# nkwangyh/CubemapSLAM

Hardware: AMD Instinct MI355X
Metric: frames/sec (extract+match+localBA) on Lafida cam0 (higher is better)
Workload: dtype u8 (extract/match), f64 (BA)

## Files before the change

### cubemapslam_amd/csrc/cms_api_ba_lm.hip

```cpp

struct BaLm {
  int iterations = 0, robust = 0;
  double delta = 0;
  int it = 0, qmax = 0, nBad = 0, done = 0, next = 0;
  double lambda = -1, ni = 2, currentChi = 0, iniChi = 0, rho = 0;
  double chi_ini = 0, chi_fin = 0, lam_fin = 0;
};

static bool ba_stopped(const volatile uint8_t* stop) { return stop && *stop; }

static int ba_enqueue_iter_start(cms_ba* b, const BaLm& st) {
  hipStream_t s = b->stream;
  const int cur = b->cur;
  ba_errors(b, cur, st.robust, st.delta, 0);
  hipLaunchKernelGGL(k_ba_lin_points, dim3(b->nblk_p), dim3(128), 0, s, b->d, (const double*)b->d_poses[cur],
                     (const double*)b->d_pts[cur], st.robust, st.delta, b->d_Hll, b->d_bl, b->d_Hpl);
  hipLaunchKernelGGL(k_ba_lin_poses, dim3(b->K, BA_POSE_CHUNKS), dim3(256), 0, s, b->d, (const double*)b->d_poses[cur],
                     (const double*)b->d_pts[cur], st.robust, st.delta, b->d_pose_partial);
  if (b->np > 0)
    hipLaunchKernelGGL(k_ba_pose_finish, dim3(b->np), dim3(64), 0, s, b->np, (const double*)b->d_pose_partial, b->d_Hpp, b->d_bp);
  if (st.it == 0) {
    HIPCHK(hipMemsetAsync(b->d_scal + 3, 0, sizeof(double), s));
    hipLaunchKernelGGL(k_ba_maxdiag, dim3(64), dim3(256), 0, s, b->np, b->P, (const double*)b->d_Hpp, (const double*)b->d_Hll, b->d_scal + 3);
  }
  HIPCHK(hipMemcpyAsync(b->h_pin, b->d_scal, 4 * sizeof(double), hipMemcpyDeviceToHost, s));
  return CMS_OK;
}
static void ba_finish_iter_start(cms_ba* b, BaLm& st) {
  st.currentChi = b->h_pin[0];
  st.iniChi = st.currentChi;
  if (st.it == 0) { st.chi_ini = st.iniChi; st.lambda = 1e-5 * b->h_pin[3]; st.ni = 2; st.nBad = 0; }
  st.rho = 0; st.qmax = 0;
// ... 95 lines not shown
      ++nact;
    }
    if (nact == 0) break;
    for (int w = 0; w < n; ++w) {
      if (stepped[w] < 0) continue;
      HIPCHK(hipStreamSynchronize(bas[w]->stream));
      if (stepped[w] == 0) ba_finish_iter_start(bas[w], st[w]);
      else ba_finish_trial(bas[w], st[w], stop);
    }
  }
  HIPCHK(hipGetLastError());
  return CMS_OK;
}

static bool ba_can_batch(cms_ba** bas, int n) {
  const bool single_old = ba_knobs().single_host_lm;
  if (n < (single_old ? 2 : 1) || n > BA_MAX_GROUP) return false;
  for (int w = 0; w < n; ++w) if (!bas[w]->solve_blk || bas[w]->device != bas[0]->device) return false;
  return true;
}
static int ba_group_reserve(cms_ba* owner, int n) {
  if (owner->grp_cap >= n) return CMS_OK;
  if (owner->grp_items_host) ba_pin_give(owner->device, owner->grp_items_host, owner->grp_pin_bytes[0]);
  if (owner->grp_scal_host) ba_pin_give(owner->device, owner->grp_scal_host, owner->grp_pin_bytes[1]);
  if (owner->grp_lm_host) ba_pin_give(owner->device, owner->grp_lm_host, owner->grp_pin_bytes[2]);
  owner->grp_items_host = nullptr; owner->grp_scal_host = nullptr; owner->grp_lm_host = nullptr;
  owner->grp_cap = 0;
  const int cap = std::max(n, 8);
  { char* q = nullptr; int rc = ba_alloc(owner, &q, (size_t)cap * sizeof(BaItem)); if (rc) return rc; owner->grp_items_dev = q; }
  { int rc = ba_alloc(owner, &owner->grp_scal_dev, (size_t)cap * 8); if (rc) return rc; }
  { char* q = nullptr; int rc = ba_alloc(owner, &q, (size_t)cap * sizeof(BaLmDev)); if (rc) return rc; owner->grp_lm_dev = q; }
  HIPCHK(ba_pin_take(owner->device, (size_t)cap * sizeof(BaItem), &owner->grp_items_host, &owner->grp_pin_bytes[0]));
  HIPCHK(ba_pin_take(owner->device, (size_t)cap * 8 * sizeof(double), (void**)&owner->grp_scal_host, &owner->grp_pin_bytes[1]));
  HIPCHK(ba_pin_take(owner->device, (size_t)cap * sizeof(BaLmDev), &owner->grp_lm_host, &owner->grp_pin_bytes[2]));
  n = cap;
  owner->grp_cap = n;
  return CMS_OK;
}
static bool ba_all_sp(cms_ba** bas, int n) {
  for (int w = 0; w < n; ++w) if (bas[w]->sp.R <= 0) return false;
  return true;
}
static bool ba_use_se(cms_ba** bas, int n) {
  if (ba_knobs().host_lm) return false;
  for (int w = 0; w < n; ++w) if (bas[w]->se.nchunks <= 0 || bas[w]->det_points) return false;
  return true;
}
static bool ba_use_te(cms_ba** bas, int n) {
  if (ba_knobs().trial_points || !ba_use_se(bas, n)) return false;
  for (int w = 0; w < n; ++w) if (bas[w]->se.Rt <= 0) return false;
  return true;
}
static int ba_device_cus(int dev) {
  static std::mutex mu;
  static int cus_of[64] = {0};
  int cus = 256;
  std::lock_guard<std::mutex> lk(mu);
  if (dev >= 0 && dev < 64) {
    if (cus_of[dev] == 0) { hipDeviceProp_t pr; cus_of[dev] = hipGetDeviceProperties(&pr, dev) == hipSuccess && pr.multiProcessorCount > 0 ? pr.multiProcessorCount : 256; }
    cus = cus_of[dev];
  }
  return cus;
}
static int ba_group_ranges(cms_ba** bas, int n) {
  const int cus = ba_device_cus(bas[0]->device);
  int R = BA_SE_RANGES;
  static const int reserve = [] { const char* v = getenv("CMS_BA_RESERVE_CUS"); return v ? std::max(0, atoi(v)) : 0; }();
// ... 64 lines not shown
        HIPCHK(hipMemsetAsync(b->d_se_bp_partial, 0, (size_t)b->np * 6 * sizeof(double), g->stream));
      }
      b->gsum_clean = false;
    }
  }
  static_assert(sizeof(BaItem) % 16 == 0, "BaItem is copied in 16-byte words");
  static const bool items_by_copy_engine = getenv("CMS_BA_ITEMS_COPY_ENGINE") != nullptr;
  if (items_by_copy_engine) HIPCHK(hipMemcpyAsync(g->grp_items_dev, items, (size_t)n * sizeof(BaItem), hipMemcpyHostToDevice, g->stream));
  else {
    const int n16 = (int)((size_t)n * sizeof(BaItem) / 16);
    hipLaunchKernelGGL(k_copy16, dim3((n16 + 63) / 64), dim3(64), 0, g->stream, (uint4*)g->grp_items_dev, (const uint4*)items, n16);
  }
  HIPCHK(hipGetLastError());
  return CMS_OK;
}
static int ba_optimize_stage_batched(cms_ba** bas, int n, std::vector<BaLm>& st, const volatile uint8_t* stop) {
  cms_ba* g = bas[0];
  hipStream_t s = g->stream;
  const BaItem* ditems = reinterpret_cast<const BaItem*>(g->grp_items_dev);
  int max_e = 0, max_p = 0, max_K = 0, max_np = 0, max_chunks = 0, max_P = 0, max_R = 0, max_spt = 64, max_pairs = 0;
  size_t lds = 0, sp_lds = 0;
  const bool all_sp = ba_all_sp(bas, n);
  for (int w = 0; w < n; ++w) {
    max_R = std::max(max_R, bas[w]->sp.R); max_spt = std::max(max_spt, bas[w]->sp_threads); max_pairs = std::max(max_pairs, bas[w]->npairs);
    sp_lds = std::max(sp_lds, bas[w]->sp_lds);
    max_e = std::max(max_e, bas[w]->nblk_e); max_p = std::max(max_p, bas[w]->nblk_p); max_K = std::max(max_K, bas[w]->K);
    max_np = std::max(max_np, bas[w]->np); max_chunks = std::max(max_chunks, bas[w]->nchunks); max_P = std::max(max_P, bas[w]->P);
    lds = std::max(lds, bas[w]->blk_lds);
  }
  int rc = CMS_OK;
  {
    BaLmDev* hlm0 = reinterpret_cast<BaLmDev*>(g->grp_lm_host);
    for (int w = 0; w < n; ++w) memset(&hlm0[w], 0, sizeof(BaLmDev));
    hipLaunchKernelGGL(kb_ba_lm_load, dim3((n + 63) / 64), dim3(64), 0, s, ditems, n, st[0].robust ? 1 : 0);
  }
  BaDyn dyn{};
  memset(&dyn, 0, sizeof(dyn));
  dyn.robust = st[0].robust; dyn.delta = st[0].delta; dyn.chi2_th = 5.991; dyn.set_level = 0;
  for (;;) {
    int n_iter = 0, n_trial = 0;
    for (int w = 0; w < n; ++w) {
      dyn.phase[w] = BA_PHASE_IDLE;
      if (st[w].next == 0 && (st[w].it >= st[w].iterations || ba_stopped(stop))) st[w].next = 2;
      if (st[w].next == 0) { dyn.phase[w] = BA_PHASE_ITER; ++n_iter; }
      else if (st[w].next == 1) { dyn.phase[w] = BA_PHASE_TRIAL; ++n_trial; }
      dyn.cur[w] = (uint8_t)bas[w]->cur; dyn.first_iter[w] = st[w].it == 0; dyn.lambda[w] = st[w].lambda;
    }
    if (n_iter + n_trial == 0) break;
    if (n_iter) {
      hipLaunchKernelGGL(kb_ba_errors, dim3(max_e, 1, n), dim3(256), 0, s, ditems, dyn, (int)BA_PHASE_ITER);
      hipLaunchKernelGGL(kb_ba_reduce, dim3(1, 1, n), dim3(256), 0, s, ditems, dyn, (int)BA_PHASE_ITER);
      hipLaunchKernelGGL(kb_ba_lin_points, dim3(max_p, 1, n), dim3(128), 0, s, ditems, dyn, (int)BA_PHASE_ITER);
      hipLaunchKernelGGL(kb_ba_lin_poses, dim3(max_K, BA_POSE_CHUNKS, n), dim3(256), 0, s, ditems, dyn, (int)BA_PHASE_ITER);
      hipLaunchKernelGGL(kb_ba_pose_finish, dim3(std::max(max_np, 1), 1, n), dim3(64), 0, s, ditems, dyn, (int)BA_PHASE_ITER);
      hipLaunchKernelGGL(kb_ba_maxdiag, dim3(1, 1, n), dim3(1024), 0, s, ditems, dyn, (int)BA_PHASE_ITER);
    }
    if (n_trial) {
      if (!all_sp)
        hipLaunchKernelGGL(kb_ba_dinv, dim3((max_P + 255) / 256, 1, n), dim3(256), 0, s, ditems, dyn, (int)BA_PHASE_TRIAL);
      if (all_sp) {
        hipLaunchKernelGGL(kb_ba_schur_points, dim3(max_R, 1, n), dim3(max_spt), sp_lds, s, ditems, dyn, (int)BA_PHASE_TRIAL);
        hipLaunchKernelGGL(kb_ba_schur_reduce, dim3(max_pairs, 1, n), dim3(256), 0, s, ditems, dyn, (int)BA_PHASE_TRIAL);
      } else if (max_chunks > 0) {
        hipLaunchKernelGGL(kb_ba_schur_chunks, dim3(max_chunks, 1, n), dim3(256), 0, s, ditems, dyn, (int)BA_PHASE_TRIAL);
      }
      hipLaunchKernelGGL(kb_ba_trial_solve, dim3(1, 1, n), dim3(384), lds, s, ditems, dyn, (int)BA_PHASE_TRIAL);
      hipLaunchKernelGGL(kb_ba_trial_points, dim3(max_p, 1, n), dim3(128), 0, s, ditems, dyn, (int)BA_PHASE_TRIAL);
      hipLaunchKernelGGL(kb_ba_reduce2, dim3(1, 1, n), dim3(256), 0, s, ditems, dyn, (int)BA_PHASE_TRIAL);
    }
    HIPCHK(hipStreamSynchronize(s));
    for (int w = 0; w < n; ++w) {
      if (dyn.phase[w] == BA_PHASE_IDLE) continue;
      memcpy(bas[w]->h_pin, g->grp_scal_host + 8 * w, 8 * sizeof(double));
      if (dyn.phase[w] == BA_PHASE_ITER) ba_finish_iter_start(bas[w], st[w]);
      else ba_finish_trial(bas[w], st[w], stop);
    }
  }
  HIPCHK(hipGetLastError());
  return CMS_OK;
}
static int ba_optimize_stage_batched_dev(cms_ba** bas, int n, std::vector<BaLm>& st, const volatile uint8_t* stop) {
  cms_ba* g = bas[0];
  hipStream_t s = g->stream;
  const BaItem* ditems = reinterpret_cast<const BaItem*>(g->grp_items_dev);
  int max_e = 0, max_p = 0, max_K = 0, max_np = 0, max_chunks = 0, max_P = 0, max_R = 0, max_spt = 64, max_pairs = 0, max_it = 0;
  size_t lds = 0, sp_lds = 0;
  const bool all_sp = ba_all_sp(bas, n);
  for (int w = 0; w < n; ++w) {
    max_R = std::max(max_R, bas[w]->sp.R); max_spt = std::max(max_spt, bas[w]->sp_threads); max_pairs = std::max(max_pairs, bas[w]->npairs);
    sp_lds = std::max(sp_lds, bas[w]->sp_lds);
    max_e = std::max(max_e, bas[w]->nblk_e); max_p = std::max(max_p, bas[w]->nblk_p); max_K = std::max(max_K, bas[w]->K);
    max_np = std::max(max_np, bas[w]->np); max_chunks = std::max(max_chunks, bas[w]->nchunks); max_P = std::max(max_P, bas[w]->P);
    lds = std::max(lds, bas[w]->blk_lds);
    max_it = std::max(max_it, st[w].iterations);
  }
  BaLmDev* hlm = reinterpret_cast<BaLmDev*>(g->grp_lm_host);
  for (int w = 0; w < n; ++w) {
    BaLmDev& L = hlm[w];
    memset(&L, 0, sizeof(L));
    L.lambda = st[w].lambda; L.ni = st[w].ni; L.it = st[w].it; L.iterations = st[w].iterations; L.nBad = st[w].nBad; L.done = st[w].done;
    L.cur = bas[w]->cur;
    L.next = (st[w].it >= st[w].iterations || ba_stopped(stop)) ? 2 : 0;
  }
  hipLaunchKernelGGL(kb_ba_lm_load, dim3((n + 63) / 64), dim3(64), 0, s, ditems, n, st[0].robust ? 1 : 0);
  BaDyn dyn{};
  memset(&dyn, 0, sizeof(dyn));
  dyn.robust = st[0].robust; dyn.delta = st[0].delta; dyn.chi2_th = 5.991; dyn.set_level = 0; dyn.dev_lm = 1; dyn.fold_finish = 1;
  bool first_round = false;
  for (int w = 0; w < n; ++w) first_round = first_round || st[w].it == 0;
  const BaGroupMode gm = ba_group_mode(bas, n);
  const bool use_se = gm.use_se, use_te = gm.use_te;
  bool iter_phase = true;
  const bool use_s3 = gm.use_s3;
  int s3_threads = 64; size_t lds3 = 0;
  for (int w = 0; w < n; ++w) { s3_threads = std::max(s3_threads, ba_s3_threads(bas[w]->np)); lds3 = std::max(lds3, bas[w]->blk3_lds); }
  {
    static const int solve_kb = [] { const char* v = getenv("CMS_BA_SOLVE_LDS_KB"); return v ? atoi(v) : 0; }();
    if (solve_kb > 0) lds3 = std::max(lds3, std::min((size_t)solve_kb * 1024, (size_t)BA_LDS_CEILING));
  }
  int max_seR = 0, max_np2 = 0, max_Rt = 0; size_t se_lds = 0, te_lds = 0, rm_lds = 0;
  const int se_waves = gm.se_waves;
  bool any_runs = false, any_rw0 = false, any_rw1 = false;
  for (int w = 0; w < n; ++w) {
    const BaSe& gs = bas[w]->grp_se;
    if (gm.run_wg) { any_rw0 = any_rw0 || gs.n_rmA > 0; any_rw1 = any_rw1 || gs.n_rm > gs.n_rmA; }
    max_seR = std::max(max_seR, gs.R_rm + gs.R); max_np2 = std::max(max_np2, gs.npairs2); se_lds = std::max(se_lds, bas[w]->se_lds_fixed);
    any_runs = any_runs || gs.R_rm > 0;
    if (gs.R_rm > 0) rm_lds = std::max(rm_lds, bas[w]->rm_lds);
    max_Rt = std::max(max_Rt, gs.Rt); te_lds = std::max(te_lds, ((size_t)24 * bas[w]->K + 6 * (size_t)std::max(bas[w]->np, 1)) * sizeof(double));
  }
  se_lds += (size_t)se_waves * ((size_t)64 * 18 * sizeof(double) + 64 * sizeof(int));
  se_lds = std::max(se_lds, rm_lds);
  const int se_threads = 64 * se_waves;
  const size_t rw_lds = ba_rw_lds(std::max(max_K, 1));
  const int rw_units0 = std::max(8, std::min(BA_RW_CUTS, ba_device_cus(bas[0]->device) * ba_knobs().rw_waves_cu0 / std::max(n, 1)));
  const int rw_units1 = std::max(8, std::min(BA_RW_CUTS, ba_device_cus(bas[0]->device) * ba_knobs().rw_waves_cu1 / std::max(n, 1)));
  const bool fused = gm.fused;
  const bool solve_reduces = fused && (gm.gsum || (!ba_knobs().separate_reduce && max_seR <= ba_knobs().solve_reduce_max));
  dyn.fused_lin = fused ? 1 : 0;
  {
    static const bool no_presum = getenv("CMS_BA_NO_SOLVE_PRESUM") != nullptr;
    const size_t need = lds3 + (size_t)max_np2 * 42 * sizeof(double);
    if (use_s3 && solve_reduces && !gm.gsum && !no_presum && need <= BA_LDS_CEILING) { dyn.solve_presum = 1; lds3 = need; }
  }
  const bool first_pass = fused && use_te && first_round && !ba_knobs().separate_first_pass;
  dyn.fold_reduce = (use_te && !ba_knobs().separate_reduce2 && ba_knobs().dup == 0) ? 1 : 0;
  int k = 0;
  const int pk = g->prof_kernel;
  const int dup = ba_knobs().dup;
  auto bracket = [&](int id, int which) {
    if (pk != id) return;
    const size_t i = 2 * (size_t)k + which;
    while (g->prof_ev.size() <= i) { hipEvent_t e = nullptr; if (hipEventCreate(&e) != hipSuccess) return; g->prof_ev.push_back(e); }
    hipEventRecord(g->prof_ev[i], s);
  };
  auto enqueue_round = [&]() {
      if (first_round && first_pass) {
        bracket(1, 0);
        hipLaunchKernelGGL(kb_ba_first_pass, dim3(max_Rt, 1, n), dim3(BA_TE_THREADS), te_lds, s, ditems, dyn, (int)BA_PHASE_ITER);
        bracket(1, 1);
        iter_phase = false;
      } else if (first_round) {
        hipLaunchKernelGGL(kb_ba_errors, dim3(max_e, 1, n), dim3(256), 0, s, ditems, dyn, (int)BA_PHASE_ITER);
        hipLaunchKernelGGL(kb_ba_reduce, dim3(1, 1, n), dim3(256), 0, s, ditems, dyn, (int)BA_PHASE_ITER);
      }
      first_round = false;
      if (iter_phase) {
        const int npb = (max_P + 255) / 256;
        bracket(1, 0);
        hipLaunchKernelGGL(kb_ba_lin, dim3(npb + max_K * BA_POSE_CHUNKS, 1, n), dim3(256), 0, s, ditems, dyn, (int)BA_PHASE_ITER, npb);
        if (dup == 1) hipLaunchKernelGGL(kb_ba_lin, dim3(npb + max_K * BA_POSE_CHUNKS, 1, n), dim3(256), 0, s, ditems, dyn, (int)BA_PHASE_ITER, npb);
        bracket(1, 1);
        bracket(2, 0);
        hipLaunchKernelGGL(kb_ba_maxdiag, dim3(1, 1, n), dim3(1024), 0, s, ditems, dyn, (int)BA_PHASE_ITER);
        bracket(2, 1);
      }
      if (fused) iter_phase = false;
      if (!all_sp && !use_se)
        hipLaunchKernelGGL(kb_ba_dinv, dim3((max_P + 255) / 256, 1, n), dim3(256), 0, s, ditems, dyn, (int)BA_PHASE_TRIAL);
      if (use_se) {
// ... 33 lines not shown
        bracket(4, 1);
      } else if (max_chunks > 0) {
        hipLaunchKernelGGL(kb_ba_schur_chunks, dim3(max_chunks, 1, n), dim3(256), 0, s, ditems, dyn, (int)BA_PHASE_TRIAL);
      }
      bracket(5, 0);
      if (use_s3 && solve_reduces && dyn.solve_presum) {
        hipLaunchKernelGGL(kb_ba_trial_solve3rp, dim3(1, 1, n), dim3(s3_threads), lds3, s, ditems, dyn, (int)BA_PHASE_TRIAL);
      } else if (use_s3 && solve_reduces) {
        hipLaunchKernelGGL(kb_ba_trial_solve3r, dim3(1, 1, n), dim3(s3_threads), lds3, s, ditems, dyn, (int)BA_PHASE_TRIAL);
        if (dup == 5) hipLaunchKernelGGL(kb_ba_trial_solve3r, dim3(1, 1, n), dim3(s3_threads), lds3, s, ditems, dyn, (int)BA_PHASE_TRIAL);
      } else if (use_s3) {
        hipLaunchKernelGGL(kb_ba_trial_solve3, dim3(1, 1, n), dim3(s3_threads), lds3, s, ditems, dyn, (int)BA_PHASE_TRIAL);
        if (dup == 5) hipLaunchKernelGGL(kb_ba_trial_solve3, dim3(1, 1, n), dim3(s3_threads), lds3, s, ditems, dyn, (int)BA_PHASE_TRIAL);
      } else {
        hipLaunchKernelGGL(kb_ba_trial_solve, dim3(1, 1, n), dim3(384), lds, s, ditems, dyn, (int)BA_PHASE_TRIAL);
        if (dup == 5) hipLaunchKernelGGL(kb_ba_trial_solve, dim3(1, 1, n), dim3(384), lds, s, ditems, dyn, (int)BA_PHASE_TRIAL);
      }
      bracket(5, 1);
      bracket(6, 0);
      if (use_te) {
        hipLaunchKernelGGL(kb_ba_trial_edges, dim3(max_Rt, 1, n), dim3(BA_TE_THREADS), te_lds, s, ditems, dyn, (int)BA_PHASE_TRIAL);
        if (dup == 6) hipLaunchKernelGGL(kb_ba_trial_edges, dim3(max_Rt, 1, n), dim3(BA_TE_THREADS), te_lds, s, ditems, dyn, (int)BA_PHASE_TRIAL);
      } else {
        hipLaunchKernelGGL(kb_ba_trial_points, dim3(max_p, 1, n), dim3(128), 0, s, ditems, dyn, (int)BA_PHASE_TRIAL);
        if (dup == 6) hipLaunchKernelGGL(kb_ba_trial_points, dim3(max_p, 1, n), dim3(128), 0, s, ditems, dyn, (int)BA_PHASE_TRIAL);
      }
      bracket(6, 1);
      bracket(7, 0);
      if (!dyn.fold_reduce) hipLaunchKernelGGL(kb_ba_reduce2, dim3(1, 1, n), dim3(256), 0, s, ditems, dyn, (int)BA_PHASE_TRIAL);
      bracket(7, 1);
      ++k;
  };
  const volatile BaLmDev* vh = reinterpret_cast<const volatile BaLmDev*>(hlm);
  hipError_t werr = hipSuccess;
  for (long spins = 0;;) {
    bool any = false;
    for (int w = 0; w < n; ++w) any = any || vh[w].next != 2;
    if (!any || (k > 0 && ba_stopped(stop))) break;
    if (k - vh[0].rounds < (stop ? 1 : 2)) { enqueue_round(); spins = 0; continue; }
    if (spins < 256) std::this_thread::yield();
    else std::this_thread::sleep_for(std::chrono::microseconds(20));
    if ((++spins & 0xFFF) == 0 && hipStreamQuery(s) != hipErrorNotReady) {
      werr = hipStreamSynchronize(s);
      if (werr != hipSuccess || k - vh[0].rounds >= 2) { if (werr == hipSuccess) werr = hipErrorUnknown; break; }
    }
  }
  const hipError_t serr = hipStreamSynchronize(s);
  HIPCHK(werr);
  HIPCHK(serr);
  HIPCHK(hipGetLastError());
  if (pk > 0)
    for (int r = 0; r < k && 2 * (size_t)r + 1 < g->prof_ev.size(); ++r) {
      float ms = 0;
      if (hipEventElapsedTime(&ms, g->prof_ev[2 * r], g->prof_ev[2 * r + 1]) == hipSuccess) { g->prof_ms += ms; ++g->prof_launches; }
    }
  for (int w = 0; w < n; ++w) {
    const BaLmDev& L = hlm[w];
    BaLm& t = st[w];
    t.lambda = L.lambda; t.ni = L.ni; t.currentChi = L.currentChi; t.iniChi = L.iniChi; t.rho = L.rho; t.it = L.it; t.qmax = L.qmax;
    t.nBad = L.nBad; t.done = L.done; t.next = 2;
    if (L.done > 0 || L.it > 0) { t.chi_ini = L.chi_ini; t.chi_fin = L.chi_fin; t.lam_fin = L.lam_fin; }
    if (L.next == 1 && L.qmax > 0 && ba_stopped(stop)) {
      ++t.done; t.chi_ini = L.chi_ini; t.chi_fin = L.currentChi; t.lam_fin = L.lambda;
    }
    bas[w]->cur = L.cur;
  }
  return CMS_OK;
}

static int ba_classify_batched(cms_ba** bas, int n, int set_level, std::vector<int>& counts) {
  cms_ba* g = bas[0];
  hipStream_t s = g->stream;
  BaDyn dyn{};
  memset(&dyn, 0, sizeof(dyn));
  dyn.chi2_th = 5.991; dyn.set_level = set_level;
  int max_e = 0;
  for (int w = 0; w < n; ++w) {
    dyn.phase[w] = BA_PHASE_CLASSIFY; dyn.cur[w] = (uint8_t)bas[w]->cur;
    max_e = std::max(max_e, bas[w]->nblk_e);
  }
  const BaItem* ditems = reinterpret_cast<const BaItem*>(g->grp_items_dev);
  hipLaunchKernelGGL(kb_ba_classify, dim3(max_e, 1, n), dim3(256), 0, s, ditems, dyn, (int)BA_PHASE_CLASSIFY);
  hipLaunchKernelGGL(kb_ba_counts_publish, dim3((n + 63) / 64), dim3(64), 0, s, ditems, n);
  HIPCHK(hipStreamSynchronize(s));
  const BaLmDev* hlm = reinterpret_cast<const BaLmDev*>(g->grp_lm_host);
  counts.resize(n);
  for (int w = 0; w < n; ++w) counts[w] = hlm[w].n_out[set_level ? 0 : 1];
  return CMS_OK;
}

static int ba_optimize_group(cms_ba** bas, int n, int its_robust, int its_final, const volatile uint8_t* stop, cms_ba_stats* stats);
extern "C" int cms_ba_optimize_many(cms_ba** bas, int n, int its_robust, int its_final, const volatile uint8_t* stop, cms_ba_stats* stats) {
  if (!bas || n < 1) return cms_fail(CMS_ERR_ARG, "cms_ba_optimize_many: bad argument");
  for (int w = 0; w < n; ++w) if (!bas[w]) return cms_fail(CMS_ERR_ARG, "null ba");
  auto kind = [&](int w) {
    const cms_ba* b = bas[w];
    int k = b->device * 8 + (b->fast_plan ? 4 : 0) + (b->se.nchunks > 0 ? 2 : 0) + (b->deterministic ? 1 : 0);
    if (b->deterministic) k += 1024 * (1 + (b->det_points ? 1 : 0) + 2 * (b->rm_lds > 0 ? 1 : 0) + 4 * std::max(0, std::min(15, b->se_waves)) + 64 * b->det_ranges);
    return k;
  };
  bool one = n <= BA_MAX_GROUP;
  for (int w = 1; w < n && one; ++w) one = kind(w) == kind(0);
  if (one) return ba_optimize_group(bas, n, its_robust, its_final, stop, stats);
  std::vector<char> done(n, 0);
  int rc_all = CMS_OK;
  for (int w0 = 0; w0 < n; ++w0) {
    if (done[w0]) continue;
    std::vector<cms_ba*> grp; std::vector<int> idx;
    for (int w = w0; w < n && (int)grp.size() < BA_MAX_GROUP; ++w)
      if (!done[w] && kind(w) == kind(w0)) { grp.push_back(bas[w]); idx.push_back(w); done[w] = 1; }
    std::vector<cms_ba_stats> gs(grp.size());
    const int rc = ba_optimize_group(grp.data(), (int)grp.size(), its_robust, its_final, stop, gs.data());
    if (stats) for (size_t i = 0; i < idx.size(); ++i) stats[idx[i]] = gs[i];
    if (rc < 0) return rc;
    if (rc != CMS_OK) rc_all = rc;
  }
  return rc_all;
// ... 11 lines not shown
  };
  for (int w = 0; w < n; ++w) { HIPCHK(hipSetDevice(bas[w]->device)); HIPCHK(ba_order_behind_setup(bas[w])); }
  if (!batched)
    for (int w = 0; w < n; ++w)
      if (bas[w]->async_pending) { HIPCHK(ba_wait_stream(bas[w]->stream)); bas[w]->async_pending = false; }
  if (batched) {
    HIPCHK(hipSetDevice(bas[0]->device));
    for (int w = 0; w < n; ++w) {
      if (bas[w]->async_pending && bas[w]->stream != bas[0]->stream) { HIPCHK(ba_wait_stream(bas[w]->stream)); bas[w]->async_pending = false; }
    }
    if (bas[0]->async_pending && bas[0]->own_stream) { HIPCHK(ba_wait_stream(bas[0]->stream)); bas[0]->async_pending = false; }
    tick("uploads-waited");
    int rcg = ba_group_reserve(bas[0], n);
    if (rcg) return rcg;
    rcg = ba_upload_items(bas, n);
    if (rcg) return rcg;
    for (int w = 0; w < n; ++w) { bas[w]->async_pending = true; bas[w]->grp_stream = bas[0]->stream; }
    tick("items");
  }
  std::vector<cms_ba_stats> local(n);
  for (int w = 0; w < n; ++w) memset(&local[w], 0, sizeof(cms_ba_stats));
  if (ba_stopped(stop)) {
    if (batched) for (int w = 0; w < n; ++w) bas[w]->gsum_clean = bas[w]->grp_se.gsum != 0;
    if (stats) memcpy(stats, local.data(), n * sizeof(cms_ba_stats));
    return 1;
  }
  const double delta = std::sqrt(5.991);
  std::vector<BaLm> st(n);
  for (int w = 0; w < n; ++w) { st[w] = BaLm(); st[w].iterations = its_robust; st[w].robust = 1; st[w].delta = delta; }
  const bool host_lm = ba_knobs().host_lm;
  for (int w = 0; w < n; ++w)
    if (bas[w]->se_only && (!batched || host_lm || !ba_use_se(bas, n)))
      return cms_fail(CMS_ERR_UNSUPPORTED, "cms_ba_optimize: the window carries only the edge-major work list but another kernel path was selected");
  int rc = batched ? (host_lm ? ba_optimize_stage_batched(bas, n, st, stop) : ba_optimize_stage_batched_dev(bas, n, st, stop)) : ba_optimize_stage_many(bas, n, st, stop);
  if (rc) return rc;
  tick("stage1");
  for (int w = 0; w < n; ++w) {
    local[w].iterations_done[0] = st[w].done; local[w].chi2_initial[0] = st[w].chi_ini; local[w].chi2_final[0] = st[w].chi_fin;
    local[w].lambda_final[0] = st[w].lam_fin;
  }
  std::vector<std::vector<uint8_t>> flags(n);
  std::vector<int> counts(n, 0);
  auto classify = [&](int set_level) -> int {
    if (batched) return ba_classify_batched(bas, n, set_level, counts);
    for (int w = 0; w < n; ++w) {
      cms_ba* b = bas[w];
      HIPCHK(hipSetDevice(b->device));
      flags[w].resize(b->E);
      hipLaunchKernelGGL(k_ba_classify, dim3(b->nblk_e), dim3(256), 0, b->stream, b->d, (const double*)b->d_poses[b->cur],
                         (const double*)b->d_pts[b->cur], 5.991, set_level, b->d_flags);
      HIPCHK(hipMemcpyAsync(flags[w].data(), b->d_flags, b->E, hipMemcpyDeviceToHost, b->stream));
    }
    for (int w = 0; w < n; ++w) HIPCHK(hipStreamSynchronize(bas[w]->stream));
    for (int w = 0; w < n; ++w) { counts[w] = 0; for (int e = 0; e < bas[w]->E; ++e) counts[w] += flags[w][e]; }
    return CMS_OK;
  };
  if (!ba_stopped(stop)) {
    rc = classify(1);
    if (rc) return rc;
    for (int w = 0; w < n; ++w) local[w].n_outliers_mid = counts[w];
    tick("classified");
    for (int w = 0; w < n; ++w) { st[w] = BaLm(); st[w].iterations = its_final; st[w].robust = 0; st[w].delta = delta; }
    rc = batched ? (host_lm ? ba_optimize_stage_batched(bas, n, st, stop) : ba_optimize_stage_batched_dev(bas, n, st, stop)) : ba_optimize_stage_many(bas, n, st, stop);
    if (rc) return rc;
    for (int w = 0; w < n; ++w) {
      local[w].iterations_done[1] = st[w].done; local[w].chi2_initial[1] = st[w].chi_ini; local[w].chi2_final[1] = st[w].chi_fin;
      local[w].lambda_final[1] = st[w].lam_fin;
    }
    tick("stage2");
  }
  rc = classify(0);
  if (rc) return rc;
  tick("classified");
  if (call_timing) fprintf(stderr, "[cms_ba_optimize_many] %d windows:%s\n", n, t_log.c_str());
  for (int w = 0; w < n; ++w) local[w].n_outliers_final = counts[w];
  if (stats) memcpy(stats, local.data(), n * sizeof(cms_ba_stats));
  if (batched)
    for (int w = 0; w < n; ++w) { bas[w]->async_pending = false; bas[w]->grp_stream = nullptr; bas[w]->gsum_clean = bas[w]->grp_se.gsum != 0; }
  return CMS_OK;
}

extern "C" int cms_ba_optimize(cms_ba* b, int its_robust, int its_final, const volatile uint8_t* stop, cms_ba_stats* st) {
  if (!b) return cms_fail(CMS_ERR_ARG, "null ba");
  return cms_ba_optimize_many(&b, 1, its_robust, its_final, stop, st);
}
```

### cubemapslam_amd/csrc/cms_ba_wrappers.hip

```cpp
#include <hip/hip_runtime.h>
#include <stdint.h>

#define BA_MAX_GROUP 64
struct BaLmDev {
  double lambda, ni, currentChi, iniChi, rho, chi_ini, chi_fin, lam_fin;
  int it, iterations, qmax, nBad, done, next, cur, rounds;
  int n_out[2], pad[2];
};
struct BaItem {
  BaDev d;
  double* poses[2]; double* pts[2];
  double* Hll; double* bl; double* Hpl; double* Hpp; double* bp; double* pose_partial; double* Dinv; double* db;
  double* chunk_sum; double* x; double* partial; double* scal;
  double* hscal;
  const int2* chunk_range; const int2* tup; const int* pair_of_block; const int* pair_chunk_off;
  uint8_t* flags;
  int nblk_e, nblk_p, nchunks, block_free;
  BaSp sp;
  BaSe se;
  BaLmDev* lm; BaLmDev* hlm;
};
template <class T> struct BaGP {
  BA_AS1 T* p;
  __device__ __forceinline__ BaGP() {}
  __device__ __forceinline__ BaGP(T* q) : p((BA_AS1 T*)q) {}
  __device__ __forceinline__ operator T*() const { return (T*)p; }
  __device__ __forceinline__ BA_AS1 T& operator[](size_t i) const { return p[i]; }
  __device__ __forceinline__ BA_AS1 T* operator->() const { return p; }
};
struct BaGP2 {
  BaGP<double> a, b;
  __device__ __forceinline__ BaGP<double> operator[](int i) const { BaGP<double> r; r.p = i ? b.p : a.p; return r; }
};
struct BaItemG {
  BaDevG d;
  BaGP2 poses, pts;
  BaGP<double> Hll, bl, Hpl, Hpp, bp, pose_partial, Dinv, db, chunk_sum, x, partial, scal, hscal;
  BaGP<const int2> chunk_range, tup;
  BaGP<const int> pair_of_block, pair_chunk_off;
  BaGP<uint8_t> flags;
  int nblk_e, nblk_p, nchunks, block_free;
  BaSpG sp; BaSeG se;
  BaGP<BaLmDev> lm, hlm;
  __device__ __forceinline__ BaItemG(const BaItem& t)
      : d(t.d), Hll(t.Hll), bl(t.bl), Hpl(t.Hpl), Hpp(t.Hpp), bp(t.bp), pose_partial(t.pose_partial), Dinv(t.Dinv), db(t.db), chunk_sum(t.chunk_sum), x(t.x),
        partial(t.partial), scal(t.scal), hscal(t.hscal), chunk_range(t.chunk_range), tup(t.tup), pair_of_block(t.pair_of_block),
        pair_chunk_off(t.pair_chunk_off), flags(t.flags), nblk_e(t.nblk_e), nblk_p(t.nblk_p), nchunks(t.nchunks), block_free(t.block_free), sp(t.sp), se(t.se),
        lm(t.lm), hlm(t.hlm) {
    poses.a = BaGP<double>(t.poses[0]); poses.b = BaGP<double>(t.poses[1]); pts.a = BaGP<double>(t.pts[0]); pts.b = BaGP<double>(t.pts[1]);
  }
};
struct BaDyn {
  double lambda[BA_MAX_GROUP];
  uint8_t phase[BA_MAX_GROUP], cur[BA_MAX_GROUP], first_iter[BA_MAX_GROUP];
  int robust, set_level;
  double delta, chi2_th;
  int dev_lm, fold_finish;
  int fused_lin, fold_reduce;
  int solve_presum, pad_;
};
enum { BA_PHASE_IDLE = 0, BA_PHASE_ITER = 1, BA_PHASE_TRIAL = 2, BA_PHASE_CLASSIFY = 3 };

extern "C" __global__ void __launch_bounds__(256)
k_ba_errors(BaDev d, const double* poses, const double* pts, int robust, double delta, double* partial) {
  ba_errors_body(blockIdx.x, gridDim.x, d, poses, pts, robust, delta, partial);
}
extern "C" __global__ void __launch_bounds__(256)
k_ba_reduce(const double* partial, int n, double* out, int add) { ba_reduce_body(blockIdx.x, gridDim.x, partial, n, out, add); }
extern "C" __global__ void __launch_bounds__(128)
k_ba_lin_points(BaDev d, const double* poses, const double* pts, int robust, double delta, double* Hll, double* bl, double* Hpl) {
  ba_lin_points_body(blockIdx.x, gridDim.x, d, poses, pts, robust, delta, Hll, bl, Hpl);
}
extern "C" __global__ void __launch_bounds__(256)
k_ba_lin_poses(BaDev d, const double* poses, const double* pts, int robust, double delta, double* pose_partial) {
  ba_lin_poses_body(blockIdx.x, gridDim.x, d, poses, pts, robust, delta, pose_partial);
}
extern "C" __global__ void __launch_bounds__(64)
k_ba_pose_finish(int np, const double* pose_partial, double* Hpp, double* bp) { ba_pose_finish_body(blockIdx.x, gridDim.x, np, pose_partial, Hpp, bp); }
extern "C" __global__ void __launch_bounds__(256)
k_ba_maxdiag(int np, int P, const double* Hpp, const double* Hll, double* out) { ba_maxdiag_body(blockIdx.x, gridDim.x, np, P, Hpp, Hll, out); }
extern "C" __global__ void __launch_bounds__(256)
k_ba_dinv(int P, const double* Hll, const double* bl, double lambda, double* Dinv, double* db) {
  ba_dinv_body(blockIdx.x, gridDim.x, P, Hll, bl, lambda, Dinv, db);
}
extern "C" __global__ void __launch_bounds__(256)
k_ba_schur_chunks(BaDev d, const int2* chunk_range, const int2* tup, const double* Hpl, const double* Dinv, const double* db, double* chunk_sum) {
  ba_schur_chunks_body(blockIdx.x, gridDim.x, d, chunk_range, tup, Hpl, Dinv, db, chunk_sum);
}
extern "C" __global__ void __launch_bounds__(BA_SP_MAX_THREADS + BA_SP_STAGERS) __attribute__((amdgpu_waves_per_eu(1, 3)))
k_ba_schur_points(BaDev d, BaSp sp, const double* Hpl, const double* Dinv, const double* db) { ba_schur_points_body(blockIdx.x, d, sp, Hpl, Dinv, db); }
extern "C" __global__ void __launch_bounds__(256)
k_ba_schur_reduce(BaSp sp, double* pair_sum) { ba_schur_reduce_body(blockIdx.x, sp, pair_sum); }
// ... 285 lines not shown
    for (int i = threadIdx.x; i < 6 * it.d.np; i += blockDim.x) {
      double sum = 0.0;
      for (int r = 0; r < n; ++r)
        sum += __longlong_as_double((long long)__hip_atomic_load(reinterpret_cast<BA_AS1 unsigned long long*>(it.se.partial) + ((size_t)r * 6 * it.d.np + i), __ATOMIC_RELAXED, __HIP_MEMORY_SCOPE_AGENT));
      m = fmax(m, fabs(sum));
    }
  } else
  for (int i = threadIdx.x; i < 6 * it.d.np; i += blockDim.x)
    m = fmax(m, fabs(__longlong_as_double((long long)__hip_atomic_exchange(reinterpret_cast<unsigned long long*>(pose_diag + i), 0ull, __ATOMIC_RELAXED, __HIP_MEMORY_SCOPE_AGENT))));
  if (threadIdx.x == 0) m = fmax(m, __longlong_as_double((long long)atomicExch(pt_max, 0ull)));
  for (int o = 32; o > 0; o >>= 1) m = fmax(m, __shfl_xor(m, o));
  __syncthreads();
  if ((threadIdx.x & 63) == 0) sh2[threadIdx.x >> 6] = m;
  __syncthreads();
  if (threadIdx.x == 0) {
    double mx = 0;
    for (int i = 0; i < (int)(blockDim.x >> 6); ++i) mx = fmax(mx, sh2[i]);
    it.scal[0] = chi; it.hscal[0] = chi; it.scal[3] = mx; it.hscal[3] = mx;
    atomicExch(ticket, 0);
    if (dyn.dev_lm) ba_lm_after_iter(it.lm, it.hlm, chi, mx);
  }
}
__device__ __forceinline__ void kb_ba_reduce2_window(const BaItem* __restrict__ items, const BaDyn& dyn, int phase) {
  BA_ITEM(phase, 1)
  ba_reduce2_body(0, 1, it.partial, it.se.Rt > 0 ? it.se.Rt : it.nblk_p, it.scal, it.hscal);
  ba_trial_publish(it, dyn);
}
extern "C" __global__ void __launch_bounds__(256) kb_ba_reduce2(const BaItem* __restrict__ items, BaDyn dyn, int phase) {
  kb_ba_reduce2_window(items, dyn, phase);
  if (dyn.dev_lm && blockIdx.z == 0 && threadIdx.x == 0) ba_round_count(items);
}
extern "C" __global__ void __launch_bounds__(256) kb_ba_classify(const BaItem* __restrict__ items, BaDyn dyn, int phase) {
  BA_ITEM(phase, it.nblk_e)
  ba_classify_body(blockIdx.x, it.nblk_e, it.d, it.poses[cur], it.pts[cur], dyn.chi2_th, dyn.set_level, it.flags);
  const int e = blockIdx.x * blockDim.x + threadIdx.x;
  const int n = __syncthreads_count(e < it.d.E && it.flags[e] != 0);
  if (threadIdx.x == 0 && n > 0) atomicAdd((int*)&it.lm->n_out[dyn.set_level ? 0 : 1], n);
}
extern "C" __global__ void __launch_bounds__(64) kb_ba_lm_load(const BaItem* __restrict__ items, int n, int clear_counts) {
  const int w = blockIdx.x * blockDim.x + threadIdx.x;
  if (w >= n) return;
  BaLmDev L = *items[w].hlm;
  const BaLmDev old = *items[w].lm;
  L.n_out[0] = clear_counts ? 0 : old.n_out[0];
  L.n_out[1] = clear_counts ? 0 : old.n_out[1];
  *items[w].lm = L;
  reinterpret_cast<int*>(items[w].scal + 7)[0] = 0;
  items[w].scal[6] = 0.0;
  for (int i = 0; i < 6 * items[w].d.np; ++i) items[w].Hpp[i] = 0.0;
}
extern "C" __global__ void __launch_bounds__(64) kb_ba_counts_publish(const BaItem* __restrict__ items, int n) {
  const int w = blockIdx.x * blockDim.x + threadIdx.x;
  if (w >= n) return;
  items[w].hlm->n_out[0] = items[w].lm->n_out[0];
  items[w].hlm->n_out[1] = items[w].lm->n_out[1];
}
```

Measured before the change: 25110.

## Chain BA stage 1, classify and stage 2 on device without host sync

Stage 1 of the device-driven LM loop no longer ends with a host synchronize. Outlier classification is enqueued directly behind it, and stage 2 is started from a staged host snapshot through kb_ba_lm_load, so the GPU keeps running across the stage boundary. A new round-decision helper limits how many speculative rounds are queued, using remaining iterations and a drained/confirm state, which cuts redundant trailing rounds. The cost is more complex host-device state handoff: stage flags, snapshot buffers, and pinned memory three times larger, with some risk of races in the stage handoff.

```diff
diff --git a/cubemapslam_amd/csrc/cms_api_ba_lm.hip b/cubemapslam_amd/csrc/cms_api_ba_lm.hip
--- a/cubemapslam_amd/csrc/cms_api_ba_lm.hip
+++ b/cubemapslam_amd/csrc/cms_api_ba_lm.hip
@@ -1,3 +1,4 @@
+#include "cms_ba_round_bound.h"
 
 struct BaLm {
   int iterations = 0, robust = 0;
@@ -159,7 +160,7 @@
   { char* q = nullptr; int rc = ba_alloc(owner, &q, (size_t)cap * sizeof(BaLmDev)); if (rc) return rc; owner->grp_lm_dev = q; }
   HIPCHK(ba_pin_take(owner->device, (size_t)cap * sizeof(BaItem), &owner->grp_items_host, &owner->grp_pin_bytes[0]));
   HIPCHK(ba_pin_take(owner->device, (size_t)cap * 8 * sizeof(double), (void**)&owner->grp_scal_host, &owner->grp_pin_bytes[1]));
-  HIPCHK(ba_pin_take(owner->device, (size_t)cap * sizeof(BaLmDev), &owner->grp_lm_host, &owner->grp_pin_bytes[2]));
+  HIPCHK(ba_pin_take(owner->device, (size_t)3 * cap * sizeof(BaLmDev), &owner->grp_lm_host, &owner->grp_pin_bytes[2]));
   n = cap;
   owner->grp_cap = n;
   return CMS_OK;
@@ -290,13 +291,13 @@
   {
     BaLmDev* hlm0 = reinterpret_cast<BaLmDev*>(g->grp_lm_host);
     for (int w = 0; w < n; ++w) memset(&hlm0[w], 0, sizeof(BaLmDev));
-    hipLaunchKernelGGL(kb_ba_lm_load, dim3((n + 63) / 64), dim3(64), 0, s, ditems, n, st[0].robust ? 1 : 0);
+    hipLaunchKernelGGL(kb_ba_lm_load, dim3((n + 63) / 64), dim3(64), 0, s, ditems, n, st[0].robust ? 1 : 0, (const BaLmDev*)nullptr);
   }
   BaDyn dyn{};
   memset(&dyn, 0, sizeof(dyn));
   dyn.robust = st[0].robust; dyn.delta = st[0].delta; dyn.chi2_th = 5.991; dyn.set_level = 0;
   for (;;) {
-    int n_iter = 0, n_trial = 0;
+    int n_iter = 0, n_trial = 0, n_timed = 0;
     for (int w = 0; w < n; ++w) {
       dyn.phase[w] = BA_PHASE_IDLE;
       if (st[w].next == 0 && (st[w].it >= st[w].iterations || ba_stopped(stop))) st[w].next = 2;
@@ -316,17 +317,27 @@
     if (n_trial) {
       if (!all_sp)
         hipLaunchKernelGGL(kb_ba_dinv, dim3((max_P + 255) / 256, 1, n), dim3(256), 0, s, ditems, dyn, (int)BA_PHASE_TRIAL);
+      const bool timed = g->prof_kernel == 3 && (all_sp || max_chunks > 0);
+      if (timed) {
+        while (g->prof_ev.size() < 2) { hipEvent_t e = nullptr; HIPCHK(hipEventCreate(&e)); g->prof_ev.push_back(e); }
+        hipEventRecord(g->prof_ev[0], s);
+      }
       if (all_sp) {
         hipLaunchKernelGGL(kb_ba_schur_points, dim3(max_R, 1, n), dim3(max_spt), sp_lds, s, ditems, dyn, (int)BA_PHASE_TRIAL);
         hipLaunchKernelGGL(kb_ba_schur_reduce, dim3(max_pairs, 1, n), dim3(256), 0, s, ditems, dyn, (int)BA_PHASE_TRIAL);
       } else if (max_chunks > 0) {
         hipLaunchKernelGGL(kb_ba_schur_chunks, dim3(max_chunks, 1, n), dim3(256), 0, s, ditems, dyn, (int)BA_PHASE_TRIAL);
       }
+      if (timed) { hipEventRecord(g->prof_ev[1], s); n_timed = 1; }
       hipLaunchKernelGGL(kb_ba_trial_solve, dim3(1, 1, n), dim3(384), lds, s, ditems, dyn, (int)BA_PHASE_TRIAL);
       hipLaunchKernelGGL(kb_ba_trial_points, dim3(max_p, 1, n), dim3(128), 0, s, ditems, dyn, (int)BA_PHASE_TRIAL);
       hipLaunchKernelGGL(kb_ba_reduce2, dim3(1, 1, n), dim3(256), 0, s, ditems, dyn, (int)BA_PHASE_TRIAL);
     }
     HIPCHK(hipStreamSynchronize(s));
+    if (n_timed) {
+      float ms = 0;
+      if (hipEventElapsedTime(&ms, g->prof_ev[0], g->prof_ev[1]) == hipSuccess) { g->prof_ms += ms; ++g->prof_launches; }
+    }
     for (int w = 0; w < n; ++w) {
       if (dyn.phase[w] == BA_PHASE_IDLE) continue;
       memcpy(bas[w]->h_pin, g->grp_scal_host + 8 * w, 8 * sizeof(double));
@@ -337,7 +348,13 @@
   HIPCHK(hipGetLastError());
   return CMS_OK;
 }
-static int ba_optimize_stage_batched_dev(cms_ba** bas, int n, std::vector<BaLm>& st, const volatile uint8_t* stop) {
+struct BaChain {
+  int phase = 0;
+  int k0 = 0;
+  bool chained = false;
+};
+static int ba_classify_enqueue(cms_ba** bas, int n, int set_level, bool cur_from_lm, BaLmDev* snap);
+static int ba_optimize_stage_batched_dev(cms_ba** bas, int n, std::vector<BaLm>& st, const volatile uint8_t* stop, BaChain* ch = nullptr) {
   cms_ba* g = bas[0];
   hipStream_t s = g->stream;
   const BaItem* ditems = reinterpret_cast<const BaItem*>(g->grp_items_dev);
@@ -353,14 +370,19 @@
     max_it = std::max(max_it, st[w].iterations);
   }
   BaLmDev* hlm = reinterpret_cast<BaLmDev*>(g->grp_lm_host);
+  const bool ch2 = ch && ch->phase == 2;
+  BaLmDev* start = ch2 ? hlm + g->grp_cap : hlm;
+  std::vector<int> next0(n);
   for (int w = 0; w < n; ++w) {
-    BaLmDev& L = hlm[w];
+    BaLmDev& L = start[w];
     memset(&L, 0, sizeof(L));
     L.lambda = st[w].lambda; L.ni = st[w].ni; L.it = st[w].it; L.iterations = st[w].iterations; L.nBad = st[w].nBad; L.done = st[w].done;
     L.cur = bas[w]->cur;
     L.next = (st[w].it >= st[w].iterations || ba_stopped(stop)) ? 2 : 0;
-  }
-  hipLaunchKernelGGL(kb_ba_lm_load, dim3((n + 63) / 64), dim3(64), 0, s, ditems, n, st[0].robust ? 1 : 0);
+    L.stage = ch2 ? 2 : 1;
+    next0[w] = L.next;
+  }
+  hipLaunchKernelGGL(kb_ba_lm_load, dim3((n + 63) / 64), dim3(64), 0, s, ditems, n, st[0].robust ? 1 : 0, (const BaLmDev*)(ch2 ? start : nullptr));
   BaDyn dyn{};
   memset(&dyn, 0, sizeof(dyn));
   dyn.robust = st[0].robust; dyn.delta = st[0].delta; dyn.chi2_th = 5.991; dyn.set_level = 0; dyn.dev_lm = 1; dyn.fold_finish = 1;
@@ -403,7 +425,7 @@
   }
   const bool first_pass = fused && use_te && first_round && !ba_knobs().separate_first_pass;
   dyn.fold_reduce = (use_te && !ba_knobs().separate_reduce2 && ba_knobs().dup == 0) ? 1 : 0;
-  int k = 0;
+  int k = ch ? ch->k0 : 0;
   const int pk = g->prof_kernel;
   const int dup = ba_knobs().dup;
   auto bracket = [&](int id, int which) {
@@ -503,18 +525,39 @@
       ++k;
   };
   const volatile BaLmDev* vh = reinterpret_cast<const volatile BaLmDev*>(hlm);
+  std::vector<BaRoundView> view(n);
   hipError_t werr = hipSuccess;
+  bool drained = false;
   for (long spins = 0;;) {
-    bool any = false;
-    for (int w = 0; w < n; ++w) any = any || vh[w].next != 2;
-    if (!any || (k > 0 && ba_stopped(stop))) break;
-    if (k - vh[0].rounds < (stop ? 1 : 2)) { enqueue_round(); spins = 0; continue; }
+    const int rounds = vh[0].rounds;
+    for (int w = 0; w < n; ++w) {
+      view[w].iterations = st[w].iterations;
+      if (ch2 && vh[w].stage != 2) { view[w].next = next0[w]; view[w].it = st[w].it; continue; }
+      view[w].next = vh[w].next; view[w].it = vh[w].it;
+    }
+    const BaRoundDecision dec = ba_round_decide(view.data(), n, k, rounds, stop != nullptr, ba_stopped(stop), drained);
+    if (dec == BA_ROUND_DONE) break;
+    if (dec == BA_ROUND_QUEUE) { enqueue_round(); drained = false; spins = 0; continue; }
+    if (dec == BA_ROUND_CONFIRM && spins >= 64) {
+      werr = hipStreamSynchronize(s);
+      if (werr == hipSuccess && vh[0].rounds != k) werr = hipErrorUnknown;
+      if (werr != hipSuccess) break;
+      drained = true; spins = 0;
+      continue;
+    }
     if (spins < 256) std::this_thread::yield();
     else std::this_thread::sleep_for(std::chrono::microseconds(20));
     if ((++spins & 0xFFF) == 0 && hipStreamQuery(s) != hipErrorNotReady) {
       werr = hipStreamSynchronize(s);
       if (werr != hipSuccess || k - vh[0].rounds >= 2) { if (werr == hipSuccess) werr = hipErrorUnknown; break; }
-    }
+      drained = vh[0].rounds == k;
+    }
+  }
+  if (ch && ch->phase == 1 && werr == hipSuccess && !ba_stopped(stop)) {
+    const int rcc = ba_classify_enqueue(bas, n, 1, true, hlm + 2 * (size_t)g->grp_cap);
+    if (rcc) return rcc;
+    ch->k0 = k; ch->chained = true;
+    return CMS_OK;
   }
   const hipError_t serr = hipStreamSynchronize(s);
   HIPCHK(werr);
@@ -539,12 +582,12 @@
   return CMS_OK;
 }
 
-static int ba_classify_batched(cms_ba** bas, int n, int set_level, std::vector<int>& counts) {
+static int ba_classify_enqueue(cms_ba** bas, int n, int set_level, bool cur_from_lm, BaLmDev* snap) {
   cms_ba* g = bas[0];
   hipStream_t s = g->stream;
   BaDyn dyn{};
   memset(&dyn, 0, sizeof(dyn));
-  dyn.chi2_th = 5.991; dyn.set_level = set_level;
+  dyn.chi2_th = 5.991; dyn.set_level = set_level; dyn.cur_from_lm = cur_from_lm ? 1 : 0;
   int max_e = 0;
   for (int w = 0; w < n; ++w) {
     dyn.phase[w] = BA_PHASE_CLASSIFY; dyn.cur[w] = (uint8_t)bas[w]->cur;
@@ -552,8 +595,15 @@
   }
   const BaItem* ditems = reinterpret_cast<const BaItem*>(g->grp_items_dev);
   hipLaunchKernelGGL(kb_ba_classify, dim3(max_e, 1, n), dim3(256), 0, s, ditems, dyn, (int)BA_PHASE_CLASSIFY);
-  hipLaunchKernelGGL(kb_ba_counts_publish, dim3((n + 63) / 64), dim3(64), 0, s, ditems, n);
-  HIPCHK(hipStreamSynchronize(s));
+  hipLaunchKernelGGL(kb_ba_counts_publish, dim3((n + 63) / 64), dim3(64), 0, s, ditems, n, snap);
+  HIPCHK(hipGetLastError());
+  return CMS_OK;
+}
+static int ba_classify_batched(cms_ba** bas, int n, int set_level, std::vector<int>& counts) {
+  cms_ba* g = bas[0];
+  const int rc = ba_classify_enqueue(bas, n, set_level, false, nullptr);
+  if (rc) return rc;
+  HIPCHK(hipStreamSynchronize(g->stream));
   const BaLmDev* hlm = reinterpret_cast<const BaLmDev*>(g->grp_lm_host);
   counts.resize(n);
   for (int w = 0; w < n; ++w) counts[w] = hlm[w].n_out[set_level ? 0 : 1];
@@ -631,10 +681,27 @@
   for (int w = 0; w < n; ++w)
     if (bas[w]->se_only && (!batched || host_lm || !ba_use_se(bas, n)))
       return cms_fail(CMS_ERR_UNSUPPORTED, "cms_ba_optimize: the window carries only the edge-major work list but another kernel path was selected");
-  int rc = batched ? (host_lm ? ba_optimize_stage_batched(bas, n, st, stop) : ba_optimize_stage_batched_dev(bas, n, st, stop)) : ba_optimize_stage_many(bas, n, st, stop);
+  BaChain chain;
+  chain.phase = 1;
+  int rc = batched ? (host_lm ? ba_optimize_stage_batched(bas, n, st, stop) : ba_optimize_stage_batched_dev(bas, n, st, stop, &chain)) : ba_optimize_stage_many(bas, n, st, stop);
   if (rc) return rc;
   tick("stage1");
-  for (int w = 0; w < n; ++w) {
+  if (chain.chained) {
+    for (int w = 0; w < n; ++w) { st[w] = BaLm(); st[w].iterations = its_final; st[w].robust = 0; st[w].delta = delta; }
+    chain.phase = 2;
+    rc = ba_optimize_stage_batched_dev(bas, n, st, stop, &chain);
+    if (rc) return rc;
+    const BaLmDev* snap = reinterpret_cast<const BaLmDev*>(bas[0]->grp_lm_host) + 2 * (size_t)bas[0]->grp_cap;
+    for (int w = 0; w < n; ++w) {
+      const BaLmDev& L = snap[w];
+      local[w].iterations_done[0] = L.done; local[w].n_outliers_mid = L.n_out[0];
+      if (L.done > 0 || L.it > 0) { local[w].chi2_initial[0] = L.chi_ini; local[w].chi2_final[0] = L.chi_fin; local[w].lambda_final[0] = L.lam_fin; }
+      local[w].iterations_done[1] = st[w].done; local[w].chi2_initial[1] = st[w].chi_ini; local[w].chi2_final[1] = st[w].chi_fin;
+      local[w].lambda_final[1] = st[w].lam_fin;
+    }
+    tick("stage2");
+  }
+  for (int w = 0; w < n && !chain.chained; ++w) {
     local[w].iterations_done[0] = st[w].done; local[w].chi2_initial[0] = st[w].chi_ini; local[w].chi2_final[0] = st[w].chi_fin;
     local[w].lambda_final[0] = st[w].lam_fin;
   }
@@ -654,7 +721,7 @@
     for (int w = 0; w < n; ++w) { counts[w] = 0; for (int e = 0; e < bas[w]->E; ++e) counts[w] += flags[w][e]; }
     return CMS_OK;
   };
-  if (!ba_stopped(stop)) {
+  if (!chain.chained && !ba_stopped(stop)) {
     rc = classify(1);
     if (rc) return rc;
     for (int w = 0; w < n; ++w) local[w].n_outliers_mid = counts[w];
diff --git a/cubemapslam_amd/csrc/cms_ba_round_bound.h b/cubemapslam_amd/csrc/cms_ba_round_bound.h
--- /dev/null
+++ b/cubemapslam_amd/csrc/cms_ba_round_bound.h
@@ -0,0 +1,26 @@
+#pragma once
+
+struct BaRoundView { int iterations, it, next; };
+
+enum BaRoundDecision {
+  BA_ROUND_DONE = 0,
+  BA_ROUND_QUEUE = 1,
+  BA_ROUND_WAIT = 2,
+  BA_ROUND_CONFIRM = 3
+};
+
+static inline BaRoundDecision ba_round_decide(const BaRoundView* v, int n, int k, int rounds, bool stop_given, bool stopped, bool drained) {
+  bool any = false;
+  for (int w = 0; w < n; ++w) any = any || v[w].next != 2;
+  if (!any || (k > 0 && stopped)) return BA_ROUND_DONE;
+  const int inflight = drained ? 0 : k - rounds;
+  if (inflight >= (stop_given ? 1 : 2)) return BA_ROUND_WAIT;
+  for (int w = 0; w < n; ++w) {
+    if (v[w].next == 2) continue;
+    const int lag = (w == 0 || drained) ? 0 : 1;
+    if (v[w].iterations - v[w].it - inflight - lag > 0) return BA_ROUND_QUEUE;
+  }
+  if (inflight > 0) return BA_ROUND_WAIT;
+  if (drained || v[0].next != 2) return BA_ROUND_QUEUE;
+  return BA_ROUND_CONFIRM;
+}
diff --git a/cubemapslam_amd/csrc/cms_ba_wrappers.hip b/cubemapslam_amd/csrc/cms_ba_wrappers.hip
--- a/cubemapslam_amd/csrc/cms_ba_wrappers.hip
+++ b/cubemapslam_amd/csrc/cms_ba_wrappers.hip
@@ -5,7 +5,8 @@
 struct BaLmDev {
   double lambda, ni, currentChi, iniChi, rho, chi_ini, chi_fin, lam_fin;
   int it, iterations, qmax, nBad, done, next, cur, rounds;
-  int n_out[2], pad[2];
+  int n_out[2];
+  int stage, pad;
 };
 struct BaItem {
   BaDev d;
@@ -57,7 +58,7 @@
   double delta, chi2_th;
   int dev_lm, fold_finish;
   int fused_lin, fold_reduce;
-  int solve_presum, pad_;
+  int solve_presum, cur_from_lm;
 };
 enum { BA_PHASE_IDLE = 0, BA_PHASE_ITER = 1, BA_PHASE_TRIAL = 2, BA_PHASE_CLASSIFY = 3 };
 
@@ -409,26 +410,38 @@
 }
 extern "C" __global__ void __launch_bounds__(256) kb_ba_classify(const BaItem* __restrict__ items, BaDyn dyn, int phase) {
   BA_ITEM(phase, it.nblk_e)
+  if (dyn.cur_from_lm) cur = it.lm->cur;
   ba_classify_body(blockIdx.x, it.nblk_e, it.d, it.poses[cur], it.pts[cur], dyn.chi2_th, dyn.set_level, it.flags);
   const int e = blockIdx.x * blockDim.x + threadIdx.x;
   const int n = __syncthreads_count(e < it.d.E && it.flags[e] != 0);
   if (threadIdx.x == 0 && n > 0) atomicAdd((int*)&it.lm->n_out[dyn.set_level ? 0 : 1], n);
 }
-extern "C" __global__ void __launch_bounds__(64) kb_ba_lm_load(const BaItem* __restrict__ items, int n, int clear_counts) {
+extern "C" __global__ void __launch_bounds__(64) kb_ba_lm_load(const BaItem* __restrict__ items, int n, int clear_counts, const BaLmDev* __restrict__ src) {
   const int w = blockIdx.x * blockDim.x + threadIdx.x;
   if (w >= n) return;
-  BaLmDev L = *items[w].hlm;
+  BaLmDev L = src ? src[w] : *items[w].hlm;
   const BaLmDev old = *items[w].lm;
   L.n_out[0] = clear_counts ? 0 : old.n_out[0];
   L.n_out[1] = clear_counts ? 0 : old.n_out[1];
+  if (src) { L.cur = old.cur; L.rounds = old.rounds; }
   *items[w].lm = L;
+  if (src) {
+    volatile BaLmDev* H = items[w].hlm;
+    const int stage = L.stage;
+    L.stage = old.stage;
+    *items[w].hlm = L;
+    __threadfence_system();
+    H->stage = stage;
+    items[w].lm->stage = stage;
+  }
   reinterpret_cast<int*>(items[w].scal + 7)[0] = 0;
   items[w].scal[6] = 0.0;
   for (int i = 0; i < 6 * items[w].d.np; ++i) items[w].Hpp[i] = 0.0;
 }
-extern "C" __global__ void __launch_bounds__(64) kb_ba_counts_publish(const BaItem* __restrict__ items, int n) {
+extern "C" __global__ void __launch_bounds__(64) kb_ba_counts_publish(const BaItem* __restrict__ items, int n, BaLmDev* __restrict__ snap) {
   const int w = blockIdx.x * blockDim.x + threadIdx.x;
   if (w >= n) return;
   items[w].hlm->n_out[0] = items[w].lm->n_out[0];
   items[w].hlm->n_out[1] = items[w].lm->n_out[1];
-}
+  if (snap) snap[w] = *items[w].lm;
+}
```

New measurement: 24870. About the same (-0.9%).
